# Berghojo/bmhrl

Measured on AMD Instinct MI355X. Metric: caption-train steps/sec, higher is better.
Workload: dtype bf16; 1 GPU; BMHRL warmstart step (BASELINE configs[1]): B=16/GPU Tv=256 Ta=800 L=30 V=10172 N=2 d_model=1024 H=4 dropout=0.1; global_batch=16, parallelism=dp1, launch=hip-graph

## Files before the change

### bmhrl_amd/csrc/elementwise.hip

```cpp
#include <cstdlib>

#include "common.h"
#include "../../include/bmhrl_hip.h"

namespace {

constexpr int ROWS_PER_BLOCK = 4;

__global__ void ln_fwd_kernel(const float* __restrict__ x, const float* __restrict__ gamma, const float* __restrict__ beta,
                              bf16_t* __restrict__ yb, long ldy, float* __restrict__ yf, float* __restrict__ mean,
                              float* __restrict__ rstd, long rows, int D) {
  const long row = (long)blockIdx.x * ROWS_PER_BLOCK + (threadIdx.x >> 6);
  if (row >= rows) return;
  const int lane = threadIdx.x & 63;
  const float* xr = x + row * D;
  float s = 0.f;
  for (int c = lane; c < D; c += 64) s += xr[c];
  const float mu = wave_sum(s) / D;
  float v = 0.f;
  for (int c = lane; c < D; c += 64) {
    const float d = xr[c] - mu;
    v += d * d;
  }
  const float rs = rsqrtf(wave_sum(v) / D + 1e-5f);
// ... 285 lines not shown
    reinterpret_cast<f32x4*>(out)[i] = v;
    if (ob) {
      bf16x4 o;
#pragma unroll
      for (int j = 0; j < 4; ++j) o[j] = (bf16_t)v[j];
      *reinterpret_cast<bf16x4*>(ob + row * ldob + 4 * c4) = o;
    }
  }
}

__global__ void embed_posenc_kernel(const int64_t* __restrict__ tok, const int64_t* __restrict__ tok2, float mix,
                                    const float* __restrict__ table, const float* __restrict__ pe, float* __restrict__ emb,
                                    float* __restrict__ out, int L, int D, long total, float scale, float p, uint64_t seed0,
                                    const uint64_t* __restrict__ seed_dev) {
  const uint64_t seed = seed0 + ((p > 0.f && seed_dev) ? seed_dev[0] : 0ull);
  for (long i = (long)blockIdx.x * blockDim.x + threadIdx.x; i < total; i += (long)gridDim.x * blockDim.x) {
    const int c = i % D;
    const long row = i / D;
    const int l = row % L;
    float e = table[tok[row] * D + c] * scale;
    if (tok2) e = e * (1.f - mix) + table[tok2[row] * D + c] * scale * mix;
    if (emb) emb[i] = e;
    float v = e + pe[(long)l * D + c];
    if (p > 0.f) v *= dropout_scale(p, seed, i);
    out[i] = v;
  }
}

__global__ void embed_bwd_kernel(const int64_t* __restrict__ tok, const int64_t* __restrict__ tok2, float mix,
                                 const float* __restrict__ dC, float* __restrict__ dtable, int D, long total, float scale) {
  for (long i = (long)blockIdx.x * blockDim.x + threadIdx.x; i < total; i += (long)gridDim.x * blockDim.x) {
    const int c = i % D;
    const long row = i / D;
    const float g = dC[i] * scale;
    if (tok2) {
      atomicAdd(dtable + tok[row] * D + c, g * (1.f - mix));
      atomicAdd(dtable + tok2[row] * D + c, g * mix);
    } else {
      atomicAdd(dtable + tok[row] * D + c, g);
    }
  }
}

__global__ void embed_bwd_ordered_kernel(const int64_t* __restrict__ tok, const int64_t* __restrict__ tok2, float mix,
                                         const float* __restrict__ dC, float* __restrict__ dtable, int D, long rows, float scale) {
  const int c = blockIdx.x * blockDim.x + threadIdx.x;
  if (c >= D) return;
  for (long row = 0; row < rows; ++row) {
    const float g = dC[row * D + c] * scale;
    if (tok2) {
      dtable[tok[row] * D + c] += g * (1.f - mix);
      dtable[tok2[row] * D + c] += g * mix;
    } else {
      dtable[tok[row] * D + c] += g;
    }
  }
}
__global__ void scatter_add_rows_ordered_kernel(const float* __restrict__ dout, const int32_t* __restrict__ src, float* __restrict__ dx,
                                                int D, long rows) {
  const int c = blockIdx.x * blockDim.x + threadIdx.x;
  if (c >= D) return;
  for (long r = 0; r < rows; ++r) {
    const int s = src[r];
    if (s >= 0) dx[(long)s * D + c] += dout[r * D + c];
  }
}

__global__ void cast_bf16_kernel(const float* __restrict__ x, long ldx, bf16_t* __restrict__ y, long ldy, long rows,
                                 int cols, float scale, float p, uint64_t seed0, const uint64_t* __restrict__ seed_dev) {
  const uint64_t seed = seed0 + ((p > 0.f && seed_dev) ? seed_dev[0] : 0ull);
  const long total = rows * cols;
  for (long i = (long)blockIdx.x * blockDim.x + threadIdx.x; i < total; i += (long)gridDim.x * blockDim.x) {
    const int c = i % cols;
    const long r = i / cols;
    float v = x[r * ldx + c] * scale;
    if (p > 0.f) v *= dropout_scale(p, seed, i);
    y[r * ldy + c] = (bf16_t)v;
  }
}

__global__ void cast_bf16_copies_kernel(const float* __restrict__ x, long ldx, bf16_t* __restrict__ y, long ldy, long rows, int cols,
                                        int copies, long copy_stride) {
  const long total = rows * cols;
  for (long i = (long)blockIdx.x * blockDim.x + threadIdx.x; i < total; i += (long)gridDim.x * blockDim.x) {
    const int c = i % cols;
    const long r = i / cols;
    const bf16_t v = (bf16_t)x[r * ldx + c];
    for (int k = 0; k < copies; ++k) y[k * copy_stride + r * ldy + c] = v;
  }
}

__global__ void cast_split3_kernel(const float* __restrict__ x, long ldx, bf16_t* __restrict__ y, long ldy, long part, int lo_slot,
                                   long rows, int cols, const float* __restrict__ x2, long ldx2, int cols2) {
  const int ct = cols + cols2;
  const long total = rows * ct;
  for (long i = (long)blockIdx.x * blockDim.x + threadIdx.x; i < total; i += (long)gridDim.x * blockDim.x) {
    const int c = i % ct;
    const long r = i / ct;
    const float v = c < cols ? x[r * ldx + c] : x2[r * ldx2 + c - cols];
    const bf16_t hi = (bf16_t)v;
    bf16_t* o = y + r * ldy + c;
    o[0] = hi;
    o[lo_slot * part] = (bf16_t)(v - (float)hi);
    o[(3 - lo_slot) * part] = hi;
  }
}

constexpr int SEG_WORDS = 6, SEG_ELEMS_PER_BLOCK = 4096;
__global__ void cast_segments_kernel(const int64_t* __restrict__ seg, int n_seg) {
  int lo = 0, hi = n_seg - 1;
  while (lo < hi) {
    const int mid = (lo + hi + 1) >> 1;
    if (seg[mid * SEG_WORDS + 5] <= (int64_t)blockIdx.x) lo = mid; else hi = mid - 1;
  }
  const int64_t* e = seg + lo * SEG_WORDS;
  const float* __restrict__ src = reinterpret_cast<const float*>(e[0]);
  const long rows = e[2], cols = e[3];
  const long ldd = e[4] <= 0 ? e[4] : (e[4] & 0xffffffffL), part = e[4] <= 0 ? 0 : (e[4] >> 32);
  const long total = rows * cols;
  const long base = ((long)blockIdx.x - e[5]) * SEG_ELEMS_PER_BLOCK;
  if (ldd <= 0) {
    float* __restrict__ dst = reinterpret_cast<float*>(e[1]);
    for (long i = base + threadIdx.x; i < base + SEG_ELEMS_PER_BLOCK && i < total; i += blockDim.x) dst[i] = src[i];
    return;
  }
  bf16_t* __restrict__ dst = reinterpret_cast<bf16_t*>(e[1]);
  if (part) {
    for (long i = base + threadIdx.x; i < base + SEG_ELEMS_PER_BLOCK && i < total; i += blockDim.x) {
      const long r = i / cols, c = i - r * cols;
      const float v = src[i];
      const bf16_t hi = (bf16_t)v;
      dst[r * ldd + c] = hi;
      dst[r * ldd + part + c] = (bf16_t)(v - (float)hi);
      dst[r * ldd + 2 * part + c] = hi;
    }
    return;
  }
  if ((cols & 3) == 0 && (ldd & 3) == 0 && ((e[0] | e[1]) & 15) == 0) {
    for (long i = base + 4 * threadIdx.x; i < base + SEG_ELEMS_PER_BLOCK && i < total; i += 4 * blockDim.x) {
      const f32x4 v = *reinterpret_cast<const f32x4*>(src + i);
      const long r = i / cols, c = i - r * cols;
      bf16x4 o;
      o[0] = (bf16_t)v[0]; o[1] = (bf16_t)v[1]; o[2] = (bf16_t)v[2]; o[3] = (bf16_t)v[3];
      *reinterpret_cast<bf16x4*>(dst + r * ldd + c) = o;
    }
  } else {
    for (long i = base + threadIdx.x; i < base + SEG_ELEMS_PER_BLOCK && i < total; i += blockDim.x) {
      const long r = i / cols, c = i - r * cols;
      dst[r * ldd + c] = (bf16_t)src[i];
    }
  }
}

__global__ void cast_colsum_kernel(const float* __restrict__ x, long ldx, bf16_t* __restrict__ y, long ldy, long rows, int cols,
                                   float scale, float p, uint64_t seed0, const uint64_t* __restrict__ seed_dev,
                                   float* __restrict__ colsum, int rows_per_block, int cgs, long group_rows, int blocks_per_group,
                                   long cs_stride) {
  __shared__ float red[1024];
  const uint64_t seed = seed0 + ((p > 0.f && seed_dev) ? seed_dev[0] : 0ull);
  const int cg = threadIdx.x % cgs, ry = threadIdx.x / cgs, rl = 256 / cgs;
  const int col = blockIdx.x * 256 + cg * 4;
  const int grp = (int)blockIdx.y / blocks_per_group;
  const long r0 = grp * group_rows + (long)((int)blockIdx.y - grp * blocks_per_group) * rows_per_block;
  rows = (grp + 1) * group_rows < rows ? (grp + 1) * group_rows : rows;
  colsum += grp * cs_stride;
  const bool vec = (ldx & 3) == 0 && (ldy & 3) == 0 && col + 4 <= cols && (((uintptr_t)x & 15) | ((uintptr_t)y & 7)) == 0;
  float acc[4] = {0.f, 0.f, 0.f, 0.f};
  long r_first = r0 + ry;
  const long r_end = r0 + rows_per_block < rows ? r0 + rows_per_block : rows;
  if (col < cols && vec) {
    for (; r_first + 3 * rl < r_end; r_first += 4 * rl) {
      f32x4 t[4];
#pragma unroll
      for (int u = 0; u < 4; ++u) t[u] = *reinterpret_cast<const f32x4*>(x + (r_first + u * rl) * ldx + col);
#pragma unroll
      for (int u = 0; u < 4; ++u) {
        const long r = r_first + u * rl;
        bf16x4 o;
#pragma unroll
        for (int j = 0; j < 4; ++j) {
          float w = t[u][j] * scale;
          if (p > 0.f) w *= dropout_scale(p, seed, (uint64_t)r * cols + col + j);
          o[j] = (bf16_t)w;
          acc[j] += (float)o[j];
        }
        *reinterpret_cast<bf16x4*>(y + r * ldy + col) = o;
      }
    }
  }
  if (col < cols) {
    for (long r = r_first; r < r_end; r += rl) {
      float v[4] = {0.f, 0.f, 0.f, 0.f};
      if (vec) {
        const f32x4 t = *reinterpret_cast<const f32x4*>(x + r * ldx + col);
        v[0] = t[0]; v[1] = t[1]; v[2] = t[2]; v[3] = t[3];
      } else {
        for (int j = 0; j < 4 && col + j < cols; ++j) v[j] = x[r * ldx + col + j];
      }
      bf16x4 o;
#pragma unroll
      for (int j = 0; j < 4; ++j) {
        float w = v[j] * scale;
        if (p > 0.f && col + j < cols) w *= dropout_scale(p, seed, (uint64_t)r * cols + col + j);
        o[j] = (bf16_t)w;
        acc[j] += (float)o[j];
      }
      if (vec) *reinterpret_cast<bf16x4*>(y + r * ldy + col) = o;
      else for (int j = 0; j < 4 && col + j < cols; ++j) y[r * ldy + col + j] = o[j];
    }
  }
#pragma unroll
  for (int j = 0; j < 4; ++j) red[ry * (4 * cgs) + cg * 4 + j] = acc[j];
  __syncthreads();
  if ((int)threadIdx.x < 4 * cgs) {
    const int c = blockIdx.x * 256 + threadIdx.x;
    if (c < cols) {
      float t = 0.f;
      for (int k = 0; k < rl; ++k) t += red[k * (4 * cgs) + threadIdx.x];
      atomicAdd(colsum + c, t);
    }
  }
}

__global__ void colsum_bf16_kernel(const bf16_t* __restrict__ dY, long ld, float* __restrict__ db, long rows, int cols,
                                   int rows_per_block, long db_stride) {
  __shared__ float red[4][512];
  dY += (long)blockIdx.z * rows * ld;
  db += (long)blockIdx.z * db_stride;
  const int cg = threadIdx.x & 63, ry = threadIdx.x >> 6;
  const int col = blockIdx.x * 512 + cg * 8;
  const long r0 = (long)blockIdx.y * rows_per_block;
  float acc[8];
#pragma unroll
  for (int j = 0; j < 8; ++j) acc[j] = 0.f;
  if (col < cols) {
    for (long r = r0 + ry; r < r0 + rows_per_block && r < rows; r += 4) {
      const bf16x8 v = *reinterpret_cast<const bf16x8*>(dY + r * ld + col);
#pragma unroll
      for (int j = 0; j < 8; ++j) acc[j] += (float)v[j];
    }
  }
#pragma unroll
  for (int j = 0; j < 8; ++j) red[ry][cg * 8 + j] = acc[j];
  __syncthreads();
  for (int c = threadIdx.x; c < 512; c += 256) {
    const int gc = blockIdx.x * 512 + c;
    if (gc < cols) atomicAdd(db + gc, red[0][c] + red[1][c] + red[2][c] + red[3][c]);
  }
}

__device__ __forceinline__ float gate_of(const float* a_v) {
  const float a = fminf(fmaxf(a_v[0], -2.f), 2.f);
  return 1.f / (1.f + __expf(-a));
}
__global__ void gate_fwd_kernel(const float* __restrict__ cv, const float* __restrict__ ca, const float* __restrict__ a_v,
                                float* __restrict__ out, bf16_t* __restrict__ ob, long ldob, int D, long total) {
  const float g = gate_of(a_v);
  for (long i = (long)blockIdx.x * blockDim.x + threadIdx.x; i < total; i += (long)gridDim.x * blockDim.x) {
    const float v = g * cv[i] + (1.f - g) * ca[i];
    out[i] = v;
    if (ob) ob[(i / D) * ldob + (i % D)] = (bf16_t)v;
  }
}
__global__ void gate_bwd_kernel(const float* __restrict__ dout, const float* __restrict__ cv, const float* __restrict__ ca,
                                const float* __restrict__ a_v, float* __restrict__ dcv, float* __restrict__ dca,
                                float* __restrict__ da_v, long total) {
  __shared__ float red[16];
  const float a = a_v[0];
  const float g = gate_of(a_v);
  float acc = 0.f;
  for (long i = (long)blockIdx.x * blockDim.x + threadIdx.x; i < total; i += (long)gridDim.x * blockDim.x) {
    const float d = dout[i];
    dcv[i] = g * d;
    dca[i] = (1.f - g) * d;
    acc += d * (cv[i] - ca[i]);
  }
  acc = block_sum(acc, red);
  if (threadIdx.x == 0 && da_v) atomicAdd(da_v, (a >= -2.f && a <= 2.f) ? acc * g * (1.f - g) : 0.f);
}

__global__ void expand_goals_index_kernel(const int32_t* __restrict__ seg, int32_t* __restrict__ src, int B, int L) {
  const int b = blockIdx.x * blockDim.x + threadIdx.x;
  if (b >= B) return;
  bool later = false;
  for (int bb = b + 1; bb < B && !later; ++bb)
    for (int l = 0; l < L; ++l)
      if (seg[bb * L + l] != 0) { later = true; break; }
  int prev = 0;
  bool any = false;
  for (int l = 0; l < L; ++l) {
    if (seg[b * L + l] != 0) {
      for (int j = prev; j <= l; ++j) src[b * L + j] = b * L + l;
      prev = l + 1;
      any = true;
    }
  }
  const bool zero_tail = later && (any || b == 0);
  for (int j = prev; j < L; ++j) src[b * L + j] = zero_tail ? -1 : b * L + j;
}
constexpr int EG_MAXL = 1024;
constexpr int EG_MAXD = 1024;
__device__ __forceinline__ float goal_noise_z(uint64_t seed, int c) {
  const float u1 = ((hash_u32(seed, 2ull * (uint64_t)c) >> 8) + 1u) * (1.0f / 16777216.0f);
  const float u2 = (hash_u32(seed, 2ull * (uint64_t)c + 1ull) >> 8) * (1.0f / 16777216.0f);
  return sqrtf(-2.f * logf(u1)) * cosf(6.283185307179586f * u2);
}
template <bool EXPLORE>
__global__ __launch_bounds__(256) void expand_goals_kernel(const int32_t* __restrict__ seg, const float* __restrict__ x,
                                                          int32_t* __restrict__ src, float* __restrict__ out,
                                                          bf16_t* __restrict__ ob, long ldob, int B, int L, int D,
                                                          float mean_factor, float std_factor, uint64_t seed,
                                                          const uint64_t* __restrict__ seed_dev, float* __restrict__ noise_out) {
  __shared__ int s_src[EG_MAXL];
  __shared__ float s_noise[EXPLORE ? EG_MAXD : 1];
  __shared__ float red[16];
  const int b = blockIdx.x;
  if constexpr (EXPLORE) {
    const long total = (long)B * L * D;
    const bool v4 = (total & 3) == 0 && ((uintptr_t)x & 15) == 0;
    const long n4 = v4 ? total >> 2 : 0;
    const f32x4* __restrict__ x4 = reinterpret_cast<const f32x4*>(x);
    float s = 0.f, cnt = 0.f;
    for (long i0 = threadIdx.x; i0 < n4; i0 += 8 * 256) {
      f32x4 t[8];
#pragma unroll
      for (int u = 0; u < 8; ++u) {
        const long i = i0 + u * 256;
        t[u] = i < n4 ? x4[i] : f32x4{NAN, NAN, NAN, NAN};
      }
#pragma unroll
      for (int u = 0; u < 8; ++u)
#pragma unroll
        for (int e = 0; e < 4; ++e) {
          const float v = t[u][e];
          if (v == v) { s += v; cnt += 1.f; }
        }
    }
    for (long i = 4 * n4 + threadIdx.x; i < total; i += 256) {
      const float v = x[i];
      if (v == v) { s += v; cnt += 1.f; }
    }
    s = block_sum(s, red);
    cnt = block_sum(cnt, red);
    const float mean = s / cnt;
    float sq = 0.f;
    for (long i0 = threadIdx.x; i0 < n4; i0 += 8 * 256) {
      f32x4 t[8];
#pragma unroll
      for (int u = 0; u < 8; ++u) {
        const long i = i0 + u * 256;
        t[u] = i < n4 ? x4[i] : f32x4{NAN, NAN, NAN, NAN};
      }
#pragma unroll
      for (int u = 0; u < 8; ++u)
#pragma unroll
        for (int e = 0; e < 4; ++e) {
          const float v = t[u][e];
          if (v == v) sq += (v - mean) * (v - mean);
        }
    }
    for (long i = 4 * n4 + threadIdx.x; i < total; i += 256) {
      const float v = x[i];
      if (v == v) sq += (v - mean) * (v - mean);
    }
    sq = block_sum(sq, red);
    const float stdv = sqrtf(sq / cnt) / std_factor, m = mean / mean_factor;
    const uint64_t sd = seed + (seed_dev ? seed_dev[0] : 0ull);
    for (int c = threadIdx.x; c < D; c += 256) {
      const float nz = goal_noise_z(sd, c) * stdv + 0.5f * m;
      s_noise[c] = nz;
      if (noise_out && b == 0) noise_out[c] = nz;
// ... 511 lines not shown
#undef LN_BWDA
    return hip_status(hipGetLastError());
  }
#define LN_BWDP(NV_) hipLaunchKernelGGL((ln_bwd_vec_kernel<NV_, true>), gridv, block, 0, S_(stream), dy, x, gamma, mean, rstd, dx, \
                                        dx_add, dg, db, (long)rows, D, rv, workspace)
  if (nv <= 1) LN_BWDP(1); else if (nv <= 2) LN_BWDP(2); else LN_BWDP(4);
#undef LN_BWDP
  const int cg = (2 * D + 63) / 64;
  int rg = (int)((256 + cg - 1) / cg);
  const int max_rg = (int)((blocks + 3) / 4);
  if (rg > max_rg) rg = max_rg;
  if (rg < 1 || bmhrl_deterministic()) rg = 1;
  hipLaunchKernelGGL(ln_bwd_reduce_kernel, dim3(cg, rg), block, 0, S_(stream), workspace, (int)blocks, D, dgamma, dbeta);
  return hip_status(hipGetLastError());
}

extern "C" int bmhrl_layernorm_fwd_groups(const float* x, const float* gamma, const float* beta, void* y_bf16, int64_t ldy,
                                          float* y_f32, float* mean, float* rstd, int64_t rows_per_group, int32_t D,
                                          int32_t groups, bmhrl_stream_t stream) {
  BMHRL_CHECK_ARG(x && gamma && beta && (y_bf16 || y_f32) && rows_per_group > 0 && D > 0 && groups >= 1 && groups <= 65535);
  const int64_t rows = rows_per_group;
  const bool vec = D % 4 == 0 && D <= 1024 && ldy % 4 == 0 && D > 128 &&
                   ((((uintptr_t)x | (uintptr_t)gamma | (uintptr_t)beta | (uintptr_t)y_f32) & 15) == 0) && (((uintptr_t)y_bf16 & 7) == 0);
  if (!vec || groups == 1) {
    for (int g = 0; g < groups; ++g) {
      const int rc = bmhrl_layernorm_fwd(x + g * rows * D, gamma + (long)g * D, beta + (long)g * D,
                                         y_bf16 ? (char*)y_bf16 + 2 * g * rows * ldy : nullptr, ldy, y_f32 ? y_f32 + g * rows * D : nullptr,
                                         mean ? mean + g * rows : nullptr, rstd ? rstd + g * rows : nullptr, rows, D, stream);
      if (rc) return rc;
    }
    return 0;
  }
  dim3 grid((unsigned)((rows + ROWS_PER_BLOCK - 1) / ROWS_PER_BLOCK), (unsigned)groups), block(256);
  const int nv = (D + 255) / 256;
#define LN_FWDG(NV_) hipLaunchKernelGGL((ln_fwd_vec_kernel<NV_, 1>), grid, block, 0, S_(stream), x, gamma, beta, (bf16_t*)y_bf16, \
                                        (long)ldy, y_f32, mean, rstd, (long)rows, D)
  if (nv <= 1) LN_FWDG(1); else if (nv <= 2) LN_FWDG(2); else LN_FWDG(4);
#undef LN_FWDG
  return hip_status(hipGetLastError());
}

extern "C" int bmhrl_layernorm_bwd_groups(const float* dy, const float* x, const float* gamma, const float* mean,
                                          const float* rstd, float* dx, const float* dx_add, float* dgamma, float* dbeta,
                                          int64_t rows_per_group, int32_t D, int32_t groups, bmhrl_stream_t stream) {
  BMHRL_CHECK_ARG(dy && x && gamma && mean && rstd && dx && rows_per_group > 0 && D > 0 && D <= 64 * LN_MAXC && groups >= 1 &&
                  groups <= 65535);
  const int64_t rows = rows_per_group;
  int rv; long blocks;
  ln_bwd_ws_plan(rows, D, &rv, &blocks);
  static const long atomic_max = getenv("BMHRL_LN_ATOMIC_BLOCKS") ? atol(getenv("BMHRL_LN_ATOMIC_BLOCKS")) : 128;
  const bool vec = D % 4 == 0 && D <= 1024 &&
                   ((((uintptr_t)dy | (uintptr_t)x | (uintptr_t)gamma | (uintptr_t)dx | (uintptr_t)dx_add) & 15) == 0);
  if (!vec || groups == 1 || blocks > atomic_max || bmhrl_deterministic()) {
    for (int g = 0; g < groups; ++g) {
      const int rc = bmhrl_layernorm_bwd(dy + g * rows * D, x + g * rows * D, gamma + (long)g * D, mean + g * rows, rstd + g * rows,
                                         dx + g * rows * D, dx_add ? dx_add + g * rows * D : nullptr,
                                         dgamma ? dgamma + (long)g * D : nullptr, dbeta ? dbeta + (long)g * D : nullptr, rows, D, stream);
      if (rc) return rc;
    }
    return 0;
  }
  dim3 gridv((unsigned)blocks, (unsigned)groups), block(256);
  const int nv = (D + 255) / 256;
#define LN_BWDG(NV_) hipLaunchKernelGGL((ln_bwd_vec_kernel<NV_, false>), gridv, block, 0, S_(stream), dy, x, gamma, mean, rstd, dx, \
                                        dx_add, dgamma, dbeta, (long)rows, D, rv, (float*)nullptr)
  if (nv <= 1) LN_BWDG(1); else if (nv <= 2) LN_BWDG(2); else LN_BWDG(4);
#undef LN_BWDG
  return hip_status(hipGetLastError());
}

extern "C" int bmhrl_add_posenc(const float* a, const float* b, const float* pe, float* out, void* out_bf16, int64_t ldob,
                                int32_t B, int32_t S, int32_t D, float dropout_p, uint64_t seed, const uint64_t* seed_dev,
                                bmhrl_stream_t stream) {
  BMHRL_CHECK_ARG(a && pe && out && B > 0 && S > 0 && D > 0);
  const long total = (long)B * S * D;
  const uintptr_t al = (uintptr_t)a | (uintptr_t)b | (uintptr_t)pe | (uintptr_t)out;
  if (D % 4 == 0 && (al & 15) == 0 && (!out_bf16 || (ldob % 4 == 0 && ((uintptr_t)out_bf16 & 7) == 0))) {
    hipLaunchKernelGGL(add_posenc_vec4_kernel, dim3(grid_for(total / 4)), dim3(256), 0, S_(stream), a, b, pe, out, (bf16_t*)out_bf16,
                       (long)ldob, S, D / 4, total / 4, dropout_p, seed, seed_dev);
    return hip_status(hipGetLastError());
  }
  hipLaunchKernelGGL(add_posenc_kernel, dim3(grid_for(total)), dim3(256), 0, S_(stream), a, b, pe, out, (bf16_t*)out_bf16,
                     (long)ldob, S, D, total, dropout_p, seed, seed_dev);
  return hip_status(hipGetLastError());
}

extern "C" int bmhrl_embed_posenc(const int64_t* tok, const int64_t* tok2, float mix, const float* table, const float* pe,
                                  float* emb_out, float* out, int32_t B, int32_t L, int32_t D, float scale,
                                  float dropout_p, uint64_t seed, const uint64_t* seed_dev, bmhrl_stream_t stream) {
  BMHRL_CHECK_ARG(tok && table && pe && out && B > 0 && L > 0 && D > 0);
  const long total = (long)B * L * D;
  hipLaunchKernelGGL(embed_posenc_kernel, dim3(grid_for(total)), dim3(256), 0, S_(stream), tok, tok2, mix, table, pe,
                     emb_out, out, L, D, total, scale, dropout_p, seed, seed_dev);
  return hip_status(hipGetLastError());
}

extern "C" int bmhrl_embed_bwd(const int64_t* tok, const int64_t* tok2, float mix, const float* dC, float* dtable,
                               int32_t B, int32_t L, int32_t D, float scale, bmhrl_stream_t stream) {
  BMHRL_CHECK_ARG(tok && dC && dtable && B > 0 && L > 0 && D > 0);
  const long total = (long)B * L * D;
  if (bmhrl_deterministic())
    hipLaunchKernelGGL(embed_bwd_ordered_kernel, dim3((unsigned)((D + 63) / 64)), dim3(64), 0, S_(stream), tok, tok2, mix, dC, dtable,
                       D, (long)B * L, scale);
  else
    hipLaunchKernelGGL(embed_bwd_kernel, dim3(grid_for(total)), dim3(256), 0, S_(stream), tok, tok2, mix, dC, dtable, D,
                       total, scale);
  return hip_status(hipGetLastError());
}

extern "C" int bmhrl_cast_bf16(const float* x, int64_t ldx, void* y, int64_t ldy, int64_t rows, int32_t cols, float scale,
                               float dropout_p, uint64_t seed, const uint64_t* seed_dev, bmhrl_stream_t stream) {
  BMHRL_CHECK_ARG(x && y && rows > 0 && cols > 0 && ldy >= cols && ldx >= cols);
  hipLaunchKernelGGL(cast_bf16_kernel, dim3(grid_for(rows * cols)), dim3(256), 0, S_(stream), x, (long)ldx, (bf16_t*)y,
                     (long)ldy, (long)rows, cols, scale, dropout_p, seed, seed_dev);
  return hip_status(hipGetLastError());
}

extern "C" int bmhrl_cast_bf16_copies(const float* x, int64_t ldx, void* y, int64_t ldy, int64_t rows, int32_t cols,
                                      int32_t copies, int64_t copy_stride, bmhrl_stream_t stream) {
  BMHRL_CHECK_ARG(x && y && rows > 0 && cols > 0 && ldy >= cols && ldx >= cols && copies >= 1 && (copies == 1 || copy_stride >= rows * ldy));
  hipLaunchKernelGGL(cast_bf16_copies_kernel, dim3(grid_for(rows * cols)), dim3(256), 0, S_(stream), x, (long)ldx, (bf16_t*)y,
                     (long)ldy, (long)rows, cols, copies, (long)copy_stride);
  return hip_status(hipGetLastError());
}

extern "C" int bmhrl_cast_colsum_bf16_groups(const float* x, int64_t ldx, void* y, int64_t ldy, int64_t rows, int32_t cols,
                                             float scale, float dropout_p, uint64_t seed, const uint64_t* seed_dev,
                                             float* colsum, int64_t group_rows, int64_t colsum_stride, bmhrl_stream_t stream);

extern "C" int bmhrl_cast_split3_bf16(const float* x, int64_t ldx, void* y, int64_t ldy, int64_t part, int32_t lo_slot,
                                      int64_t rows, int32_t cols, const float* x2, int64_t ldx2, int32_t cols2,
                                      bmhrl_stream_t stream) {
  BMHRL_CHECK_ARG(x && y && rows > 0 && cols > 0 && ldx >= cols && ldy >= 3 * part && (lo_slot == 1 || lo_slot == 2));
  if (!x2) cols2 = 0;
  BMHRL_CHECK_ARG(cols2 >= 0 && part >= cols + cols2 && (!x2 || ldx2 >= cols2));
  hipLaunchKernelGGL(cast_split3_kernel, dim3(grid_for(rows * (cols + cols2))), dim3(256), 0, S_(stream), x, (long)ldx, (bf16_t*)y,
                     (long)ldy, (long)part, lo_slot, (long)rows, cols, x2, (long)ldx2, cols2);
  return hip_status(hipGetLastError());
}

extern "C" int bmhrl_cast_colsum_bf16(const float* x, int64_t ldx, void* y, int64_t ldy, int64_t rows, int32_t cols, float scale,
                                      float dropout_p, uint64_t seed, const uint64_t* seed_dev, float* colsum,
                                      bmhrl_stream_t stream) {
  return bmhrl_cast_colsum_bf16_groups(x, ldx, y, ldy, rows, cols, scale, dropout_p, seed, seed_dev, colsum, rows, 0, stream);
}

extern "C" int bmhrl_cast_colsum_bf16_groups(const float* x, int64_t ldx, void* y, int64_t ldy, int64_t rows_all, int32_t cols,
                                             float scale, float dropout_p, uint64_t seed, const uint64_t* seed_dev,
                                             float* colsum, int64_t group_rows, int64_t colsum_stride, bmhrl_stream_t stream) {
  BMHRL_CHECK_ARG(x && y && colsum && rows_all > 0 && cols > 0 && ldy >= cols && ldx >= cols);
  BMHRL_CHECK_ARG(group_rows > 0 && rows_all % group_rows == 0);
  const int groups = (int)(rows_all / group_rows);
  const int64_t rows = group_rows;
  const int col_blocks = (cols + 255) / 256;
  int row_blocks = 512 / col_blocks;
  row_blocks = row_blocks < 1 ? 1 : (row_blocks > 128 ? 128 : row_blocks);
  if (bmhrl_deterministic()) row_blocks = 1;
  int rpb = (int)((rows + row_blocks - 1) / row_blocks);
  if (rpb < 16) rpb = 16;
  const int bpg = (int)((rows + rpb - 1) / rpb);
  dim3 grid((unsigned)col_blocks, (unsigned)(bpg * groups)), block(256);
  int cgs = 64;
  while (cgs > 1 && (cgs / 2) * 4 >= (cols < 256 ? cols : 256)) cgs /= 2;
  hipLaunchKernelGGL(cast_colsum_kernel, grid, block, 0, S_(stream), x, (long)ldx, (bf16_t*)y, (long)ldy, (long)rows_all, cols,
                     scale, dropout_p, seed, seed_dev, colsum, rpb, cgs, (long)group_rows, bpg, (long)colsum_stride);
  return hip_status(hipGetLastError());
}

extern "C" int bmhrl_cast_segments(const int64_t* segments, int32_t n_segments, int32_t n_blocks, bmhrl_stream_t stream) {
  BMHRL_CHECK_ARG(segments && n_segments > 0 && n_blocks > 0);
  hipLaunchKernelGGL(cast_segments_kernel, dim3((unsigned)n_blocks), dim3(256), 0, S_(stream), segments, n_segments);
  return hip_status(hipGetLastError());
}

extern "C" int bmhrl_colsum_bf16(const void* dY, int64_t ld, float* db, int32_t accumulate, int64_t rows, int32_t cols,
                                 bmhrl_stream_t stream) {
  BMHRL_CHECK_ARG(dY && db && rows > 0 && cols > 0);
  if (!accumulate) {
    hipError_t e = hipMemsetAsync(db, 0, sizeof(float) * cols, S_(stream));
    if (e != hipSuccess) return (int)e;
  }
  BMHRL_CHECK_ARG(ld % 8 == 0 && ((uintptr_t)dY & 15) == 0);
  const int col_blocks = (cols + 511) / 512;
  int rpb = (int)((rows * col_blocks + 511) / 512);
  if (rpb < 16) rpb = 16;
  if (bmhrl_deterministic()) rpb = (int)rows;
  dim3 grid((unsigned)col_blocks, (unsigned)((rows + rpb - 1) / rpb)), block(256);
  hipLaunchKernelGGL(colsum_bf16_kernel, grid, block, 0, S_(stream), (const bf16_t*)dY, (long)ld, db, (long)rows, cols, rpb, 0l);
  return hip_status(hipGetLastError());
}

extern "C" int bmhrl_colsum_bf16_groups(const void* dY, int64_t ld, float* db, int64_t rows_per_group, int32_t cols,
                                        int32_t groups, int64_t db_stride, bmhrl_stream_t stream) {
  BMHRL_CHECK_ARG(dY && db && rows_per_group > 0 && cols > 0 && groups >= 1 && groups <= 65535);
  BMHRL_CHECK_ARG(ld % 8 == 0 && ((uintptr_t)dY & 15) == 0);
  const int col_blocks = (cols + 511) / 512;
  int rpb = (int)((rows_per_group * groups * col_blocks + 511) / 512);
  if (rpb < 16) rpb = 16;
  if (bmhrl_deterministic()) rpb = (int)rows_per_group;
  dim3 grid((unsigned)col_blocks, (unsigned)((rows_per_group + rpb - 1) / rpb), (unsigned)groups), block(256);
  hipLaunchKernelGGL(colsum_bf16_kernel, grid, block, 0, S_(stream), (const bf16_t*)dY, (long)ld, db, (long)rows_per_group, cols, rpb,
                     (long)db_stride);
  return hip_status(hipGetLastError());
}

static int tail_table(const bmhrl_fusion_tail_params* groups, int32_t n_groups, bool bwd, TailTable& T) {
  BMHRL_CHECK_ARG(groups && (n_groups == 1 || n_groups == 2));
  for (int i = 0; i < n_groups; ++i) {
    const bmhrl_fusion_tail_params& g = groups[i];
    BMHRL_CHECK_ARG(g.gamma_ca && g.beta_ca && g.gamma_cv && g.beta_cv && g.a_v);
    (void)bwd;
    T.g[i] = g;
  }
  if (n_groups == 1) T.g[1] = T.g[0];
  return 0;
}

extern "C" int bmhrl_fusion_tail_fwd(const float* ca, const float* cv, const bmhrl_fusion_tail_params* groups, int32_t n_groups,
                                     int64_t rows_per_group, int32_t D, float* out, float* stats, void* out_bf16, int64_t ldob,
                                     bmhrl_stream_t stream) {
  BMHRL_CHECK_ARG(ca && cv && out && stats && rows_per_group > 0 && D > 0 && D <= TAIL_MAXD);
  TailTable T;
  if (int rc = tail_table(groups, n_groups, false, T)) return rc;
  const long rows = rows_per_group * n_groups;
  dim3 grid((unsigned)((rows + 3) / 4)), block(256);
  BMHRL_CHECK_ARG(!out_bf16 || ldob >= D);
  if (D <= 320) hipLaunchKernelGGL(fusion_tail_fwd_kernel<5>, grid, block, 0, S_(stream), ca, cv, T, (long)rows_per_group, n_groups, D, out, stats, (bf16_t*)out_bf16, (long)ldob);
  else hipLaunchKernelGGL(fusion_tail_fwd_kernel<8>, grid, block, 0, S_(stream), ca, cv, T, (long)rows_per_group, n_groups, D, out, stats, (bf16_t*)out_bf16, (long)ldob);
  return hip_status(hipGetLastError());
}

extern "C" int bmhrl_fusion_tail_bwd(const float* dout, const float* dout1, int64_t ldd0, int64_t ldd1, const float* ca,
                                     const float* cv, const float* stats, const bmhrl_fusion_tail_params* groups, int32_t n_groups,
                                     int64_t rows_per_group, int32_t D, float* dca, float* dcv, bmhrl_stream_t stream) {
  BMHRL_CHECK_ARG(dout && ca && cv && stats && dca && dcv && rows_per_group > 0 && D > 0 && D <= TAIL_MAXD);
  TailTable T;
  if (int rc = tail_table(groups, n_groups, true, T)) return rc;
  if (ldd0 <= 0) ldd0 = D;
  if (ldd1 <= 0) ldd1 = ldd0;
  if (!dout1) dout1 = dout + rows_per_group * ldd0;
  BMHRL_CHECK_ARG(ldd0 >= D && ldd1 >= D);
  dim3 grid((unsigned)((rows_per_group + TAIL_RPB - 1) / TAIL_RPB), (unsigned)n_groups), block(256);
  if (D <= 320) hipLaunchKernelGGL(fusion_tail_bwd_kernel<5>, grid, block, 0, S_(stream), dout, dout1, (long)ldd0, (long)ldd1, ca, cv, stats, T, (long)rows_per_group, n_groups, D, dca, dcv);
  else hipLaunchKernelGGL(fusion_tail_bwd_kernel<8>, grid, block, 0, S_(stream), dout, dout1, (long)ldd0, (long)ldd1, ca, cv, stats, T, (long)rows_per_group, n_groups, D, dca, dcv);
  return hip_status(hipGetLastError());
}

extern "C" int bmhrl_gate_fwd(const float* cv, const float* ca, const float* a_v, float* out, void* out_bf16, int64_t ldob,
                              int64_t rows, int32_t D, bmhrl_stream_t stream) {
  BMHRL_CHECK_ARG(cv && ca && a_v && out && rows > 0 && D > 0);
  const long total = rows * D;
  hipLaunchKernelGGL(gate_fwd_kernel, dim3(grid_for(total)), dim3(256), 0, S_(stream), cv, ca, a_v, out, (bf16_t*)out_bf16,
                     (long)ldob, D, total);
  return hip_status(hipGetLastError());
}

extern "C" int bmhrl_gate_bwd(const float* dout, const float* cv, const float* ca, const float* a_v, float* dcv, float* dca,
                              float* da_v, int64_t rows, int32_t D, bmhrl_stream_t stream) {
  BMHRL_CHECK_ARG(dout && cv && ca && a_v && dcv && dca && rows > 0 && D > 0);
  const long total = rows * D;
  hipLaunchKernelGGL(gate_bwd_kernel, dim3(bmhrl_deterministic() ? 1u : grid_for(total, 256, 256)), dim3(256), 0, S_(stream), dout,
                     cv, ca, a_v, dcv, dca, da_v, total);
  return hip_status(hipGetLastError());
}

extern "C" int bmhrl_expand_goals_index(const int32_t* seg, int32_t* src, int32_t B, int32_t L, bmhrl_stream_t stream) {
  BMHRL_CHECK_ARG(seg && src && B > 0 && L > 0);
  hipLaunchKernelGGL(expand_goals_index_kernel, dim3((B + 63) / 64), dim3(64), 0, S_(stream), seg, src, B, L);
  return hip_status(hipGetLastError());
}

extern "C" int bmhrl_expand_goals(const int32_t* seg, const float* x, int32_t* src, float* out, void* out_bf16, int64_t ldob,
                                  int32_t B, int32_t L, int32_t D, bmhrl_stream_t stream) {
  BMHRL_CHECK_ARG(seg && x && src && out && B > 0 && L > 0 && L <= EG_MAXL && D > 0 && (!out_bf16 || ldob >= D));
  hipLaunchKernelGGL(expand_goals_kernel<false>, dim3((unsigned)B), dim3(256), 0, S_(stream), seg, x, src, out,
                     (bf16_t*)out_bf16, (long)ldob, B, L, D, 1.f, 1.f, 0ull, (const uint64_t*)nullptr, (float*)nullptr);
  return hip_status(hipGetLastError());
}

extern "C" int bmhrl_expand_goals_explore(const int32_t* seg, const float* x, int32_t* src, float* out, void* out_bf16,
                                          int64_t ldob, int32_t B, int32_t L, int32_t D, float mean_factor, float std_factor,
                                          uint64_t seed, const uint64_t* seed_dev, float* noise_out, bmhrl_stream_t stream) {
  BMHRL_CHECK_ARG(seg && x && src && out && B > 0 && L > 0 && L <= EG_MAXL && D > 0 && D <= EG_MAXD && (!out_bf16 || ldob >= D));
  BMHRL_CHECK_ARG(mean_factor != 0.f && std_factor != 0.f && (int64_t)B * L * D < (1ll << 24));
  hipLaunchKernelGGL(expand_goals_kernel<true>, dim3((unsigned)B), dim3(256), 0, S_(stream), seg, x, src, out,
                     (bf16_t*)out_bf16, (long)ldob, B, L, D, mean_factor, std_factor, (uint64_t)seed, seed_dev, noise_out);
  return hip_status(hipGetLastError());
}

extern "C" int bmhrl_gather_rows(const float* x, const int32_t* src, float* out, void* out_bf16, int64_t ldob, int64_t rows,
                                 int32_t D, bmhrl_stream_t stream) {
  BMHRL_CHECK_ARG(x && src && out && rows > 0 && D > 0);
  const long total = rows * D;
  hipLaunchKernelGGL(gather_rows_kernel, dim3(grid_for(total)), dim3(256), 0, S_(stream), x, src, out, (bf16_t*)out_bf16,
                     (long)ldob, D, total);
  return hip_status(hipGetLastError());
}

extern "C" int bmhrl_scatter_add_rows(const float* dout, const int32_t* src, float* dx, int64_t rows, int32_t D,
                                      bmhrl_stream_t stream) {
  BMHRL_CHECK_ARG(dout && src && dx && rows > 0 && D > 0);
  const long total = rows * D;
  if (bmhrl_deterministic())
    hipLaunchKernelGGL(scatter_add_rows_ordered_kernel, dim3((unsigned)((D + 63) / 64)), dim3(64), 0, S_(stream), dout, src, dx, D,
                       (long)rows);
  else
    hipLaunchKernelGGL(scatter_add_rows_kernel, dim3(grid_for(total)), dim3(256), 0, S_(stream), dout, src, dx, D, total);
  return hip_status(hipGetLastError());
}

static int adam_step_launch(float* param, const float* grad, float* exp_avg, float* exp_avg_sq, int64_t n, float lr, float beta1,
                            float beta2, float eps, float weight_decay, int32_t step, const int32_t* step_dev, float grad_scale,
                            const float* hyper, bmhrl_stream_t stream) {
  BMHRL_CHECK_ARG(param && grad && exp_avg && exp_avg_sq && n > 0 && (step >= 1 || step_dev));
  const float bc1 = 1.f - powf(beta1, (float)step);
  const float bc2s = sqrtf(1.f - powf(beta2, (float)step));
  hipLaunchKernelGGL(adam_kernel, dim3(grid_for(n, 256, 4096)), dim3(256), 0, S_(stream), param, grad, exp_avg, exp_avg_sq,
                     (long)n, lr, beta1, beta2, eps, weight_decay, bc1, bc2s, grad_scale, step_dev, hyper);
// ... 74 lines not shown
```

Measured before the change: 213.4 steps/s (one step = one B=16 batch on one GPU; whole-job aggregate over all GPUs).

## Retune cast_colsum launch grid, block size and unroll depth

Rewrites the fused cast+column-sum kernel so block width (cgs), thread count (up to 512), and row-unroll depth (4 or 8, templated) adapt to problem shape. It targets a fixed count of about 256 blocks and caps atomic adders per column. A two-stage shared-memory reduction is added for taller blocks, and the unrolled load loop handles tails with guards plus a sched_barrier so loads are issued together. The aim is better occupancy and memory-level parallelism for this bandwidth-bound op. The cost is more register pressure and more atomics in some shapes.

```diff
diff --git a/bmhrl_amd/csrc/elementwise.hip b/bmhrl_amd/csrc/elementwise.hip
--- a/bmhrl_amd/csrc/elementwise.hip
+++ b/bmhrl_amd/csrc/elementwise.hip
@@ -461,14 +461,16 @@
   }
 }
 
-__global__ void cast_colsum_kernel(const float* __restrict__ x, long ldx, bf16_t* __restrict__ y, long ldy, long rows, int cols,
-                                   float scale, float p, uint64_t seed0, const uint64_t* __restrict__ seed_dev,
-                                   float* __restrict__ colsum, int rows_per_block, int cgs, long group_rows, int blocks_per_group,
-                                   long cs_stride) {
-  __shared__ float red[1024];
+constexpr int CAST_COLSUM_MAX_THREADS = 512;
+template <int U>
+__global__ __launch_bounds__(CAST_COLSUM_MAX_THREADS) void cast_colsum_kernel(
+    const float* __restrict__ x, long ldx, bf16_t* __restrict__ y, long ldy, long rows, int cols, float scale, float p,
+    uint64_t seed0, const uint64_t* __restrict__ seed_dev, float* __restrict__ colsum, int rows_per_block, int cgs,
+    long group_rows, int blocks_per_group, long cs_stride) {
+  __shared__ float red[4 * CAST_COLSUM_MAX_THREADS];
   const uint64_t seed = seed0 + ((p > 0.f && seed_dev) ? seed_dev[0] : 0ull);
-  const int cg = threadIdx.x % cgs, ry = threadIdx.x / cgs, rl = 256 / cgs;
-  const int col = blockIdx.x * 256 + cg * 4;
+  const int cg = threadIdx.x % cgs, ry = threadIdx.x / cgs, rl = (int)blockDim.x / cgs;
+  const int col = blockIdx.x * (4 * cgs) + cg * 4;
   const int grp = (int)blockIdx.y / blocks_per_group;
   const long r0 = grp * group_rows + (long)((int)blockIdx.y - grp * blocks_per_group) * rows_per_block;
   rows = (grp + 1) * group_rows < rows ? (grp + 1) * group_rows : rows;
@@ -478,22 +480,28 @@
   long r_first = r0 + ry;
   const long r_end = r0 + rows_per_block < rows ? r0 + rows_per_block : rows;
   if (col < cols && vec) {
-    for (; r_first + 3 * rl < r_end; r_first += 4 * rl) {
-      f32x4 t[4];
-#pragma unroll
-      for (int u = 0; u < 4; ++u) t[u] = *reinterpret_cast<const f32x4*>(x + (r_first + u * rl) * ldx + col);
-#pragma unroll
-      for (int u = 0; u < 4; ++u) {
-        const long r = r_first + u * rl;
-        bf16x4 o;
-#pragma unroll
-        for (int j = 0; j < 4; ++j) {
-          float w = t[u][j] * scale;
-          if (p > 0.f) w *= dropout_scale(p, seed, (uint64_t)r * cols + col + j);
-          o[j] = (bf16_t)w;
-          acc[j] += (float)o[j];
+    for (; r_first < r_end; r_first += (long)U * rl) {
+      f32x4 t[U];
+#pragma unroll
+      for (int u = 0; u < U; ++u) {
+        const long r = r_first + (long)u * rl;
+        t[u] = *reinterpret_cast<const f32x4*>(x + (r < r_end ? r : r_first) * ldx + col);
+      }
+      __builtin_amdgcn_sched_barrier(0);
+#pragma unroll
+      for (int u = 0; u < U; ++u) {
+        const long r = r_first + (long)u * rl;
+        if (r < r_end) {
+          bf16x4 o;
+#pragma unroll
+          for (int j = 0; j < 4; ++j) {
+            float w = t[u][j] * scale;
+            if (p > 0.f) w *= dropout_scale(p, seed, (uint64_t)r * cols + col + j);
+            o[j] = (bf16_t)w;
+            acc[j] += (float)o[j];
+          }
+          *reinterpret_cast<bf16x4*>(y + r * ldy + col) = o;
         }
-        *reinterpret_cast<bf16x4*>(y + r * ldy + col) = o;
       }
     }
   }
@@ -521,11 +529,21 @@
 #pragma unroll
   for (int j = 0; j < 4; ++j) red[ry * (4 * cgs) + cg * 4 + j] = acc[j];
   __syncthreads();
+  int nk = rl;
+  if (rl > 16) {
+    const int w = 4 * cgs, ci = threadIdx.x % w, pi = threadIdx.x / w, np = (int)blockDim.x / w;
+    float t = 0.f;
+    for (int k = pi; k < rl; k += np) t += red[k * w + ci];
+    __syncthreads();
+    red[pi * w + ci] = t;
+    __syncthreads();
+    nk = np;
+  }
   if ((int)threadIdx.x < 4 * cgs) {
-    const int c = blockIdx.x * 256 + threadIdx.x;
+    const int c = blockIdx.x * (4 * cgs) + threadIdx.x;
     if (c < cols) {
       float t = 0.f;
-      for (int k = 0; k < rl; ++k) t += red[k * (4 * cgs) + threadIdx.x];
+      for (int k = 0; k < nk; ++k) t += red[k * (4 * cgs) + threadIdx.x];
       atomicAdd(colsum + c, t);
     }
   }
@@ -1343,18 +1361,29 @@
   BMHRL_CHECK_ARG(group_rows > 0 && rows_all % group_rows == 0);
   const int groups = (int)(rows_all / group_rows);
   const int64_t rows = group_rows;
-  const int col_blocks = (cols + 255) / 256;
-  int row_blocks = 512 / col_blocks;
-  row_blocks = row_blocks < 1 ? 1 : (row_blocks > 128 ? 128 : row_blocks);
-  if (bmhrl_deterministic()) row_blocks = 1;
+  int cgs = 64;
+  while (cgs > 1 && (cgs / 2) * 4 >= (cols < 256 ? cols : 256)) cgs /= 2;
+  const bool ordered = bmhrl_deterministic();
+  constexpr int kBlocks = 256, kThreads = CAST_COLSUM_MAX_THREADS, kMaxAdders = 128;
+  if (!ordered)
+    while (cgs > 16 && ((cols + 4 * cgs - 1) / (4 * cgs)) * kMaxAdders < kBlocks) cgs /= 2;
+  const int col_blocks = (cols + 4 * cgs - 1) / (4 * cgs);
+  const int threads = ordered ? 256 : kThreads;
+  int row_blocks = (kBlocks + col_blocks - 1) / col_blocks;
+  const int64_t one_pass = (rows + 8 * (threads / cgs) - 1) / (8 * (threads / cgs));
+  if (row_blocks < one_pass) row_blocks = (int)(one_pass < kMaxAdders ? one_pass : kMaxAdders);
+  row_blocks = row_blocks < 1 ? 1 : (row_blocks > kMaxAdders ? kMaxAdders : row_blocks);
+  if (ordered) row_blocks = 1;
   int rpb = (int)((rows + row_blocks - 1) / row_blocks);
   if (rpb < 16) rpb = 16;
   const int bpg = (int)((rows + rpb - 1) / rpb);
-  dim3 grid((unsigned)col_blocks, (unsigned)(bpg * groups)), block(256);
-  int cgs = 64;
-  while (cgs > 1 && (cgs / 2) * 4 >= (cols < 256 ? cols : 256)) cgs /= 2;
-  hipLaunchKernelGGL(cast_colsum_kernel, grid, block, 0, S_(stream), x, (long)ldx, (bf16_t*)y, (long)ldy, (long)rows_all, cols,
-                     scale, dropout_p, seed, seed_dev, colsum, rpb, cgs, (long)group_rows, bpg, (long)colsum_stride);
+  const int rows_per_thread = (rpb + threads / cgs - 1) / (threads / cgs);
+  dim3 grid((unsigned)col_blocks, (unsigned)(bpg * groups)), block((unsigned)threads);
+#define CAST_COLSUM(U_) hipLaunchKernelGGL(cast_colsum_kernel<U_>, grid, block, 0, S_(stream), x, (long)ldx, (bf16_t*)y, (long)ldy, \
+                                           (long)rows_all, cols, scale, dropout_p, seed, seed_dev, colsum, rpb, cgs,              \
+                                           (long)group_rows, bpg, (long)colsum_stride)
+  if (!ordered && rows_per_thread > 4) CAST_COLSUM(8); else CAST_COLSUM(4);
+#undef CAST_COLSUM
   return hip_status(hipGetLastError());
 }
 
```

Result: no change. 213.3 steps/s (one step = one B=16 batch on one GPU; whole-job aggregate over all GPUs) (-0.1%).
